# sharph/s-rack

Hardware: AMD Instinct MI355X
Metric: voice-samples/sec @48 kHz offline render (higher is better)
Workload: dtype f32

## Files before the change

### s-rack_amd/csrc/capi.cpp

```cpp
#include <hip/hip_runtime.h>

#include <algorithm>
#include <cmath>
#include <cstdio>
#include <cstring>
#include <mutex>
#include <string>
#include <thread>
#include <vector>

#include "freeverb_params.hpp"
#include "jit.hpp"
#include "runtime.hpp"

using namespace srack;

namespace srack {
int load_srk(const uint8_t* bytes, size_t n_bytes, Graph& g);
std::vector<uint8_t> save_srk(const Graph& g);
}

struct srack_patch {
    PatchHandle h;
};
// ... 1394 lines not shown
int srack_render_info(srack_patch* p, char* buf, size_t cap)
{
    return guarded([&]() -> int {
        CHECK_HANDLE(p);
        int rc = ensure_program(p->h, p->h.prog_valid ? p->h.prog_flags : 0u);
        if (rc != SRACK_OK) return rc;
        std::string s = p->h.prog.description;
        s += tuning_knobs_note();
        const char* k = device_kernel_name(p->h);
        s += device_bus_note(p->h);
        s += device_sends_note(p->h);
        s += device_busvcf_note(p->h);
        s += device_busvca_note(p->h);
        s += device_busfx_note(p->h);
        s += device_master_note(p->h);
        s += device_waves_note(p->h);
        s += device_sequences_note(p->h);
        s += device_jit_note(p->h);
        if (k && *k) s += std::string(" kernel=") + k;
        if (buf && cap) {
            std::strncpy(buf, s.c_str(), cap - 1);
            buf[cap - 1] = 0;
        }
        return (int)s.size();
    });
}

int srack_render_kernel_source(srack_patch* p, uint32_t flags, char* buf, size_t cap)
{
    return guarded([&]() -> int {
// ... 347 lines not shown
```

### s-rack_amd/csrc/chain.hip

```cpp
#include "fused.hip.h"
#include "launch.hpp"

namespace srack {

__global__ __launch_bounds__(64) void render_ctl_gate_env(CtlWork w)
{
    if (w.port & OSC_EXACT)
        ctl_gate_env<true>(w);
    else
        ctl_gate_env<false>(w);
}

void launch_ctl_gate_env(const CtlWork& w, hipStream_t st)
{
    hipLaunchKernelGGL(render_ctl_gate_env, dim3(1), dim3(64), 0, st, w);
}

void launch_fused(uint32_t osc_port, uint32_t vcf_port, bool exact, int out_mode, bool track, const KernelArgs& ka, const ChainRoles& roles, const CtlWork& co,
                  dim3 grid, hipStream_t st)
{
    with_osc_port(osc_port, [&](auto A) { launch_chain<decltype(A)::value>(vcf_port, exact, out_mode, track, ka, roles, co, grid, st); });
}

}
```

### s-rack_amd/csrc/chain_saw.hip

```cpp
#include "chain_unit.hip.h"

namespace srack {
template void launch_chain<OSC_OUT_SAW>(uint32_t, bool, int, bool, const KernelArgs&, const ChainRoles&, const CtlWork&, dim3, hipStream_t);
}
```

### s-rack_amd/csrc/chain_sine.hip

```cpp
#include "chain_unit.hip.h"

namespace srack {
template void launch_chain<OSC_OUT_SINE>(uint32_t, bool, int, bool, const KernelArgs&, const ChainRoles&, const CtlWork&, dim3, hipStream_t);
}
```

### s-rack_amd/csrc/chain_square.hip

```cpp
#include "chain_unit.hip.h"

namespace srack {
template void launch_chain<OSC_OUT_SQUARE>(uint32_t, bool, int, bool, const KernelArgs&, const ChainRoles&, const CtlWork&, dim3, hipStream_t);
}
```

### s-rack_amd/csrc/chain_unit.hip.h

```cpp
#pragma once
#include "fused.hip.h"
#include "launch.hpp"

namespace srack {

template <uint32_t A, uint32_t F, bool E, int O>
static void launch_fused4(bool track, const KernelArgs& ka, const ChainRoles& roles, const CtlWork& co, dim3 grid, hipStream_t st)
{
    if (track)
        hipLaunchKernelGGL((render_voice_chain_track<A, F, E, O>), grid, dim3(64), 0, st, ka, roles, co);
    else
        hipLaunchKernelGGL((render_voice_chain<A, OSC_OUT_SQUARE, F, E, O>), grid, dim3(64), 0, st, ka, roles);
}

template <uint32_t A, uint32_t F>
static void launch_fused3(bool exact, int out_mode, bool track, const KernelArgs& ka, const ChainRoles& roles, const CtlWork& co, dim3 grid, hipStream_t st)
{
    if ((out_mode & kOutStats) && exact)
        launch_fused4<A, F, true, kOutStats>(track, ka, roles, co, grid, st);
    else if (out_mode & kOutStats)
        launch_fused4<A, F, false, kOutStats>(track, ka, roles, co, grid, st);
    else if (exact && out_mode == 3 && track)
        hipLaunchKernelGGL((render_voice_chain_track<A, F, true, 3>), grid, dim3(64), 0, st, ka, roles, co);
    else if (exact)
        launch_fused4<A, F, true, 0>(track, ka, roles, co, grid, st);
    else
        with_out_mode(out_mode, [&](auto O) { launch_fused4<A, F, false, O>(track, ka, roles, co, grid, st); });
}

template <uint32_t kOscAPort>
void launch_chain(uint32_t vcf_port, bool exact, int out_mode, bool track, const KernelArgs& ka, const ChainRoles& roles, const CtlWork& co, dim3 grid, hipStream_t st)
{
#ifdef SRK_WAVE_CENSUS
    if (track) (void)hipMemcpyToSymbolAsync(HIP_SYMBOL(srk_census_rec), census_rec, sizeof(*census_rec), 0, hipMemcpyHostToDevice, st);
#endif
    with_port<VCF_OUT_LP, VCF_OUT_BP, VCF_OUT_HP>(vcf_port, [&](auto F) { launch_fused3<kOscAPort, F>(exact, out_mode, track, ka, roles, co, grid, st); });
}

}
```

### s-rack_amd/csrc/folds.hip.h

```cpp
#pragma once
#include <hip/hip_runtime.h>
#include <type_traits>

#include "kernel_args.hip.h"
#include "modules.hip.h"
#include "wave.hip.h"

namespace srack {

constexpr uint32_t kMixSplit = 16;

struct MixArgs {
    const float* mixpart;
    float* mixgroup;
    float* mix;
    uint32_t T, n_waves, n_channels, n_planes;
    uint32_t mix_stride;
    uint32_t t_begin, t_end;
    int32_t channel_plane[8];
};

__global__ __launch_bounds__(256) void mix_reduce_groups(MixArgs m)
{
    const uint32_t i = m.t_begin + blockIdx.x * 256u + threadIdx.x;
    if (i >= m.t_end) return;
// ... 138 lines not shown
```

### s-rack_amd/csrc/fused.hip.h

```cpp
#pragma once
#include <hip/hip_runtime.h>
#include <type_traits>

#include "kernel_args.hip.h"
#include "launch_types.hpp"
#include "modules.hip.h"
#include "wave.hip.h"

#ifndef SRK_PRIO_AT1
#define SRK_PRIO_AT1 32
#endif
#ifndef SRK_PRIO_AT0
#define SRK_PRIO_AT0 56
#endif


namespace srack {


template <uint32_t kOscPort, bool kExact>
SRK_DEV void ctl_gate_env_body(const CtlWork& a)
{
    using namespace dev;
    const ChainRoles r{0, 0, 0, 1, 0, 2, 0};
    const int lane = threadIdx.x;
    auto row = [&](int rr) { return a.table[rr]; };
    const DevOp& ol = a.ops[r.osc_l];
    const DevOp& od = a.ops[r.adsr];
// ... 234 lines not shown
}
SRK_DEV void census_end(uint32_t* rec)
{
    if (!rec) return;
    const uint64_t t = __builtin_amdgcn_s_memrealtime();
    rec[2] = (uint32_t)t;
    rec[3] = (uint32_t)(t >> 32);
}
SRK_DEV void census_end(uint32_t* rec, const dev::Pace& p)
{
    if (rec && p.word) rec[6] = 1u | 4u | (p.key << 3) | ((p.max_lead < 255u ? p.max_lead : 255u) << 16) | ((p.mine < 255u ? p.mine : 255u) << 24);
    census_end(rec);
}
#endif

template <uint32_t kOscAPort, uint32_t kVcfPort, bool kExact, int kOut>
__global__ __launch_bounds__(64) void render_voice_chain_track(KernelArgs a, ChainRoles r, CtlWork co)
{
    using namespace dev;
    __shared__ __attribute__((aligned(16))) float mix_tile[kMixTile];
    if (blockIdx.x < a.block0) {
        __builtin_amdgcn_s_setprio(3);
#ifdef SRK_WAVE_CENSUS
        uint32_t* crec = census_begin(a.n_waves, 0xffffffffu, true, threadIdx.x);
#endif
        ctl_gate_env<kExact>(co);
#ifdef SRK_WAVE_CENSUS
        census_end(crec);
#endif
        return;
    }
    const int lane = threadIdx.x;
#ifdef SRK_WAVE_CENSUS
    uint32_t* crec = census_begin(blockIdx.x - a.block0, blockIdx.x - a.block0, false, lane);
#endif
    const WaveMap wm = wave_map(a, lane);
    const uint32_t voice = wm.voice, vc = wm.vc, V = a.V;
    const bool active = wm.active;
    auto row = [&](int rr) { return a.table[(size_t)rr * V + vc]; };
    auto parv = [&](const DevOp& op, int k) { return op.par_row[k] >= 0 ? __uint_as_float(row(op.par_row[k])) : op.par_val[k]; };
// ... 194 lines not shown
```

### s-rack_amd/csrc/launch.hpp

```cpp
#pragma once
#include <hip/hip_runtime.h>

#include <cstddef>
#include <cstdint>
#include <type_traits>

#include "kernel_args.hip.h"
#include "launch_types.hpp"

namespace srack {

struct FlatProgram;

enum class Kernel { Interp, VoiceChain, VoiceChainTrack, SeqChain, FmPair, FmPairRing, FmPairSplit, FmPairBlock, FmPairBlockX, FmPairX };

template <class Fn>
static auto with_out_mode(int out_mode, Fn&& f)
{
    switch (out_mode) {
    case 3: return f(std::integral_constant<int, 3>{});
    case 1: return f(std::integral_constant<int, 1>{});
    case 2: return f(std::integral_constant<int, 2>{});
    default: return f(std::integral_constant<int, 0>{});
    }
// ... 4 lines not shown
{
    if (port == P0)
        f(std::integral_constant<uint32_t, P0>{});
    else if (port == P1)
        f(std::integral_constant<uint32_t, P1>{});
    else
        f(std::integral_constant<uint32_t, P2>{});
}
template <class Fn>
static void with_osc_port(uint32_t port, Fn&& f)
{
    with_port<OSC_OUT_SAW, OSC_OUT_SQUARE, OSC_OUT_SINE>(port, f);
}

template <uint32_t kOscAPort>
void launch_chain(uint32_t vcf_port, bool exact, int out_mode, bool track, const KernelArgs& ka, const ChainRoles& roles, const CtlWork& co, dim3 grid, hipStream_t st);
void launch_fused(uint32_t osc_port, uint32_t vcf_port, bool exact, int out_mode, bool track, const KernelArgs& ka, const ChainRoles& roles, const CtlWork& co,
                  dim3 grid, hipStream_t st);
void launch_ctl_gate_env(const CtlWork& w, hipStream_t st);
#ifdef SRK_WAVE_CENSUS
extern uint32_t* const* census_rec;
#endif

void launch_seq(uint32_t osc_port, int out_mode, const KernelArgs& ka, const SeqRoles& r, dim3 grid, hipStream_t st);

void launch_fm_pair(Kernel kernel, bool exact, int out_mode, const KernelArgs& ka, const ChainRoles& roles, dim3 grid, hipStream_t st);
void launch_fm_pair_x(int out_mode, const KernelArgs& ka, const ChainRoles& roles, dim3 grid, hipStream_t st);
hipError_t launch_fm_block(bool x, int out_mode, const KernelArgs& ka, const ChainRoles& roles, hipStream_t st);

inline size_t interp_lds_bytes(const DevProgram& H)
{
    return ((size_t)H.n_rows + 2 + (size_t)H.n_tracks + (size_t)H.n_slots * H.tile) * 256;
}
// ... 13 lines not shown
```

### s-rack_amd/csrc/launch_types.hpp

```cpp
#pragma once
#include <cstdint>

#include "kernel_args.hip.h"

namespace srack {

struct CtlWork {
    const DevOp* ops;
    uint32_t* table;
    float* track;
    uint32_t T;
    uint32_t port;
    uint32_t* table_out;
    uint32_t n_rows;
};

constexpr int kBlkVoices = 32, kBlkSlices = 16, kBlkPer = 16, kBlkChunk = kBlkSlices * kBlkPer;

struct MasterArgs {
    const float* rows;
    const float* gain;
    float* runs;
    float* master;
    double* stats;
    uint32_t n;
    uint32_t n_buses;
    uint32_t row_channels;
    uint32_t used;
};
// ... 77 lines not shown
```

### s-rack_amd/csrc/render.hip

```cpp
#include <hip/hip_runtime.h>

#include <algorithm>
#include <cstdio>
#include <cstdlib>
#include <cstring>
#include <memory>
#include <string>
#include <type_traits>
#include <vector>

#include "busfx.hip.h"
#include "folds.hip.h"
#include "freeverb_params.hpp"
#include "jit.hpp"
#include "kernel_args.hip.h"
#include "launch.hpp"
#include "runtime.hpp"
#include "wave.hip.h"

namespace srack {


#define HIP_TRY(expr)                                                                                   \
    do {                                                                                                \
// ... 3 lines not shown
            return SRACK_ERR_DEVICE;                                                                    \
        }                                                                                               \
    } while (0)

struct Knobs {
    uint32_t want_waves = 1024;
    uint32_t chunk_max = 4096;
    uint32_t chunk_first = 1024;
    bool debug_occ = false;
    int high_prio_ctl = 1;
    int special_ctl = 1;
    int fm_split = 1;
    int fm_block = 1;
    uint32_t fm_block_chunk = 65536;
    uint32_t fm_block_min = 4096;
    int mix_aside = 0;
    int pace = 1;
    int tile_plain = 1;
    int tick = 2;
};
static const Knobs& knobs()
{
    static const Knobs k = [] {
        Knobs v;
        auto num = [](const char* name, long lo, long hi, long dflt) {
            const char* e = getenv(name);
            if (!e || !*e) return dflt;
            char* end = nullptr;
            const long x = strtol(e, &end, 10);
            if (end == e) return dflt;
            return std::min(std::max(x, lo), hi);
        };
        v.want_waves = (uint32_t)num("SRACK_WANT_WAVES", 1, 1 << 20, 1024);
        v.chunk_max = (uint32_t)num("SRACK_CHUNK_MAX", 256, 65536, 4096);
        v.chunk_first = (uint32_t)num("SRACK_CHUNK_FIRST", 32, 4096, 1024);
        v.debug_occ = getenv("SRACK_DEBUG_OCC") != nullptr;
        v.high_prio_ctl = (int)num("SRACK_CTL_HIGH_PRIO", 0, 1, 1);
        v.special_ctl = (int)num("SRACK_SPECIAL_CTL", 0, 1, 1);
        v.fm_split = (int)num("SRACK_FM_SPLIT", 0, 1, 1);
        v.fm_block = (int)num("SRACK_FM_BLOCK", 0, 1, 1);
        v.fm_block_chunk = (uint32_t)num("SRACK_FM_BLOCK_CHUNK", 256, 65536, 65536);
        v.fm_block_min = (uint32_t)num("SRACK_FM_BLOCK_MIN", 1, 65536, 4096);
        v.tick = (int)num("SRACK_TICK", 0, 2, 2);
        v.mix_aside = (int)num("SRACK_MIX_ASIDE", 0, 1, 0);
        v.pace = (int)num("SRACK_PACE", 0, 1, 1);
        v.tile_plain = (int)num("SRACK_TILE_PLAIN", 0, 1, 1);
        return v;
    }();
    return k;
}

struct DevProg {
    DevOp* d_ops = nullptr;
    uint32_t* d_table = nullptr;
    float* d_rings = nullptr;
    uint32_t* d_seqtab = nullptr;
    double* d_fv = nullptr;
    void release()
    {
// ... 21 lines not shown
    uint64_t n0 = 0;
    hipStream_t st = nullptr;
    hipEvent_t done = nullptr;
    float* d_ring = nullptr;
    size_t ring_bytes = 0;
    std::vector<uint32_t*> d_copies;
    std::vector<size_t> words;
    uint64_t slots_base = 0;
    uint32_t slots_n = 0;
};
constexpr uint32_t kPaceSlices = 16;
constexpr uint32_t kTickBatch = 256, kTickFirstBatch = 8;

struct DeviceState {
    TickSession tick;
    hipStream_t mix_stream = nullptr;
    std::vector<hipEvent_t> ev_mix;
    hipEvent_t ev_mix_done = nullptr;
    DevProg voice;
    std::vector<DevProg> ctl;
    KernelArgs* d_stage_slots = nullptr;
    size_t stage_slots_cap = 0;
    std::vector<KernelArgs> h_stage_slots;
    float* d_mixpart = nullptr;
    size_t mixpart_bytes = 0;
    float* d_mixgroup = nullptr;
    size_t mixgroup_bytes = 0;
    float* d_tracks = nullptr;
    size_t tracks_bytes = 0;
    uint32_t* d_pace = nullptr;
    float* d_stat_frames = nullptr;
    size_t stat_frames_bytes = 0;
    uint32_t* d_bus_tab = nullptr;
    uint64_t bus_revision = 0;
    float* d_bus_part = nullptr;
    size_t bus_part_bytes = 0;
    bool last_bank_lds = false;
    uint32_t last_buses = 0;
    std::shared_ptr<const JitKernel> jit[5];
    bool jit_failed = false;
    bool bank_lds[5] = {false, false, false, false, false};
    std::string jit_note;
    std::vector<std::pair<hipEvent_t, hipEvent_t>> timings;
    std::vector<hipEvent_t> pool;
    const char* kernel_name = "";
// ... 6 lines not shown

void device_release(DeviceState* d)
{
    if (!d) return;
    d->voice.release();
    for (DevProg& c : d->ctl) c.release();
    (void)hipFree(d->d_stage_slots);
    (void)hipFree(d->d_mixpart);
    (void)hipFree(d->d_mixgroup);
    (void)hipFree(d->d_tracks);
    (void)hipFree(d->d_pace);
    (void)hipFree(d->d_stat_frames);
    (void)hipFree(d->d_bus_tab);
    (void)hipFree(d->d_bus_part);
    if (d->tick.done) (void)hipEventDestroy(d->tick.done);
    for (hipEvent_t e : d->ev_mix) (void)hipEventDestroy(e);
    if (d->ev_mix_done) (void)hipEventDestroy(d->ev_mix_done);
    if (d->mix_stream) (void)hipStreamDestroy(d->mix_stream);
    (void)hipFree(d->tick.d_ring);
    for (uint32_t* c : d->tick.d_copies) (void)hipFree(c);
    for (auto& p : d->timings) {
        (void)hipEventDestroy(p.first);
        (void)hipEventDestroy(p.second);
    }
    for (auto e : d->pool) (void)hipEventDestroy(e);
    for (auto e : d->ev_chunk) (void)hipEventDestroy(e);
    if (d->ev_begin) (void)hipEventDestroy(d->ev_begin);
    if (d->ev_ready) (void)hipEventDestroy(d->ev_ready);
    if (d->ctl_stream) (void)hipStreamDestroy(d->ctl_stream);
    delete d;
}

PatchHandle::~PatchHandle()
// ... 356 lines not shown
        d->bank_lds[out_mode] = how.bank_lds;
    }
    d->last_bank_lds = d->bank_lds[out_mode];
    *out = d->jit[out_mode].get();
    *with_ctl = ctl;
    pick.name = "render_specialized";
    pick.stats_in_kernel = pick.paced = false;
    if (P.hdr.n_rings == 0 && n_waves <= 1024 && !(flags & SRACK_RENDER_EXACT_OSC)) pick.chunk = std::min(knobs().chunk_max, 2048u);
    return SRACK_OK;
}

static void launch_ctl(const FlatProgram& Cp, const KernelArgs& kc, hipStream_t st)
{
    if (Cp.fused == FUSED_CTL_GATE_ENV) {
        CtlWork w{kc.ops, kc.table, kc.frames + (size_t)Cp.ops[2].aux * kc.plane_stride, kc.T,
                  Cp.ops[0].flags & (OSC_OUT_SINE | OSC_OUT_SQUARE | OSC_OUT_SAW | OSC_EXACT), nullptr, 0u};
        launch_ctl_gate_env(w, st);
    } else if (Cp.fused == FUSED_FM_PAIR) {
        const bool exact = (Cp.render_flags & SRACK_RENDER_EXACT_OSC) != 0;
        launch_fm_pair(fm_pair_kernel(Cp.fused_variant, exact), exact, 1, kc, fm_pair_roles(Cp), dim3(1), st);
    } else {
        launch_interp(Cp, kc, st, knobs().debug_occ);
    }
}

#ifdef SRK_WAVE_CENSUS
static struct {
    uint32_t* d_rec = nullptr;
    uint32_t cap = 0, used = 0;
    std::vector<uint32_t> slots;
    std::vector<uint32_t*> where;
// ... 61 lines not shown
    float* d_bus;
    uint32_t bus_slab = 0;
    const hipStream_t st;
    int rc = SRACK_OK;
    KernelPick pick;
    const uint32_t lanes, n_waves;
    bool has_ctl = false, co_ctl = false, special_ctl = false, tick = false;
    uint32_t n_stages = 0, n_tracks = 0, kChunkMax = 0, kChunkFirst = 0, max_lag = 0, n_chunks = 0, n_ctl_launch = 0;
    uint32_t stride = 0;
    const JitKernel* special = nullptr;
    std::vector<std::pair<uint32_t, uint32_t>> chunks;
    ChainRoles roles{};
    SeqRoles seq{};
    uint32_t osc_port = 0, vcf_port = 0, seq_port = 0;
    MixArgs m{};
    bool mix_aside = false;

    Segment(PatchHandle& h_, uint32_t T_total_, uint32_t t_seg_, uint32_t T_, float* d_frames_, float* d_mix_, double* d_stats_, float* d_bus_, uint32_t flags_, hipStream_t st_)
        : h(h_), P(h_.prog.voice), d(h_.dev), tk(h_.dev->tick), V(h_.prog.voice.n_voices), C((uint32_t)h_.prog.voice.hdr.n_channels), T_total(T_total_),
          t_seg(t_seg_), T(T_), flags(flags_), d_frames(d_frames_ ? d_frames_ + (size_t)t_seg_ * h_.prog.voice.n_voices : nullptr),
          d_mix(d_mix_ ? d_mix_ + t_seg_ : nullptr), d_stats(d_stats_), d_bus(d_bus_ ? d_bus_ + t_seg_ : nullptr), st(st_), pick(pick_kernel(h_.prog, flags_, T_)), lanes(pick.lanes), n_waves((h_.prog.voice.n_voices + lanes - 1) / lanes)
    {
    }

    CtlWork ctl_work(uint32_t t_off, uint32_t len)
    {
        const FlatProgram& Cp = h.prog.ctl[0];
        return CtlWork{d->ctl[0].d_ops, d->ctl[0].d_table, d->d_tracks + (size_t)Cp.ops[2].aux * T + t_off, len,
                       Cp.ops[0].flags & (OSC_OUT_SINE | OSC_OUT_SQUARE | OSC_OUT_SAW | OSC_EXACT), nullptr, 0u};
    }
    int get_event(hipEvent_t& e)
    {
        if (!d->pool.empty()) {
            e = d->pool.back();
            d->pool.pop_back();
            return SRACK_OK;
        }
        HIP_TRY(hipEventCreate(&e));
        return SRACK_OK;
    }

    KernelArgs unit_args(uint32_t s)
    {
        KernelArgs kc{};
// ... 64 lines not shown
        KernelArgs kc = unit_args(s2);
        kc.table = tick_table(s2, x);
        kc.table_out = tick_table(s2, x + 1);
        kc.frames = tick_tracks(x);
        kc.tracks = kc.frames;
        kc.plane_stride = tk.S;
        kc.t_stride = tk.S;
        kc.T = tick_len(x);
        kc.n0 = tick_n0(x);
        return kc;
    }
    CtlWork tick_work(uint64_t x)
    {
        const FlatProgram& Cp = h.prog.ctl[0];
        return CtlWork{d->ctl[0].d_ops, tick_table(0, x), tick_tracks(x) + (size_t)Cp.ops[2].aux * tk.S, tick_len(x),
                       Cp.ops[0].flags & (OSC_OUT_SINE | OSC_OUT_SQUARE | OSC_OUT_SAW | OSC_EXACT), tick_table(0, x + 1), (uint32_t)Cp.hdr.n_rows};
    }
    int tick_upload_slots(uint64_t base)
    {
        const uint32_t fill = max_lag + 1, batch = std::max(base == 0 ? kTickFirstBatch : kTickBatch, tk.n);
        d->h_stage_slots.assign((size_t)(fill + batch) * n_stages, KernelArgs{});
        for (uint32_t s2 = 0; s2 < n_stages; s2++) {
            const uint32_t lag = (uint32_t)h.prog.ctl_lag[s2];
            if (base == 0)
                for (uint32_t g = lag; g < fill; g++) d->h_stage_slots[(size_t)g * n_stages + s2] = tick_unit_args(s2, g - lag);
            for (uint32_t i = 0; i < batch; i++) d->h_stage_slots[(size_t)(fill + i) * n_stages + s2] = tick_unit_args(s2, base + i + fill - lag);
        }
        if ((rc = upload_slots(st)) != SRACK_OK) return rc;
        tk.slots_base = base;
        tk.slots_n = batch;
        return SRACK_OK;
// ... 265 lines not shown
    }

    int voices()
    {
        if (d_mix) {
            m.mixpart = d->d_mixpart;
            m.mixgroup = d->d_mixgroup;
            m.mix = d_mix;
            m.T = stride;
            m.mix_stride = T_total;
            m.n_waves = n_waves;
            m.n_channels = C;
            m.n_planes = (uint32_t)P.hdr.n_planes;
            for (int c = 0; c < 8; c++) m.channel_plane[c] = P.hdr.channel_plane[c];
        }
        mix_aside = d_mix && n_chunks > 1 && knobs().mix_aside;
        if (mix_aside) {
            if (!d->mix_stream) HIP_TRY(hipStreamCreateWithFlags(&d->mix_stream, hipStreamNonBlocking));
            if (!d->ev_mix_done) HIP_TRY(hipEventCreateWithFlags(&d->ev_mix_done, hipEventDisableTiming));
            while (d->ev_mix.size() < n_chunks) {
                hipEvent_t e = nullptr;
                HIP_TRY(hipEventCreateWithFlags(&e, hipEventDisableTiming));
                d->ev_mix.push_back(e);
            }
        }
        const bool paced = pick.paced, exact = (flags & SRACK_RENDER_EXACT_OSC) != 0;
        if (paced && !d->d_pace) HIP_TRY(hipMalloc(&d->d_pace, sizeof(uint32_t) * dev::kPaceKeys * kPaceSlices));
        for (uint32_t k = 0; k < n_chunks; k++) {
            const uint32_t t_off = chunks[k].first, len = chunks[k].second;
            KernelArgs ka{};
            if (paced) {
                if (k % kPaceSlices == 0)
                    HIP_TRY(hipMemsetAsync(d->d_pace, 0, sizeof(uint32_t) * dev::kPaceKeys * std::min(kPaceSlices, n_chunks - k), st));
                ka.pace = d->d_pace + (size_t)(k % kPaceSlices) * dev::kPaceKeys;
            }
            ka.ops = d->voice.d_ops;
            ka.prog = P.hdr;
            ka.table = d->voice.d_table;
            ka.rings = d->voice.d_rings;
            ka.seqtab = d->voice.d_seqtab;
            ka.fv = d->voice.d_fv;
            ka.frames = d_frames ? d_frames + (size_t)t_off * V : nullptr;
            ka.mixpart = d_mix ? d->d_mixpart + t_off : nullptr;
            ka.tracks = tick ? tick_tracks(tk.c + k) : has_ctl ? d->d_tracks + t_off : nullptr;
            ka.plane_stride = (uint64_t)T_total * V;
            ka.t_stride = stride;
            ka.V = V;
            ka.T = len;
            ka.n_waves = n_waves;
// ... 4 lines not shown
            if (fold_rows) {
                ka.frames = d->d_stat_frames;
                ka.plane_stride = (uint64_t)fold_rows * V;
            }
            CtlWork co{};
            if (tick && co_ctl) {
                co = tick_work(tk.c + k + 1);
                ka.block0 = 1;
            } else if (tick) {
                ka.block0 = n_stages;
                ka.ctl_slots = d->d_stage_slots + (size_t)(max_lag + 1 + (tk.c + k - tk.slots_base)) * n_stages;
            } else if (co_ctl && k + 1 < n_chunks) {
                co = ctl_work(chunks[k + 1].first, chunks[k + 1].second);
                ka.block0 = 1;
            }
            if (has_ctl && !co_ctl && !(special && special_ctl)) HIP_TRY(hipStreamWaitEvent(st, d->ev_chunk[k], 0));
            if (!tick && special && special_ctl && k + max_lag + 1 < n_ctl_launch) {
                ka.block0 = n_stages;
                ka.ctl_slots = d->d_stage_slots + (size_t)(k + max_lag + 1) * n_stages;
            }
            hipEvent_t e0 = nullptr, e1 = nullptr;
            const bool timed = h.timing_armed;
            if (timed) {
                if ((rc = get_event(e0)) != SRACK_OK || (rc = get_event(e1)) != SRACK_OK) return rc;
                HIP_TRY(hipEventRecord(e0, st));
            }
            const int out_mode = (ka.frames ? 1 : 0) | (ka.mixpart ? 2 : 0);
            if (special) {
                if ((rc = jit_launch(*special, ka, n_waves + ka.block0, st)) != SRACK_OK) return rc;
            } else {
                switch (pick.kernel) {
                case Kernel::VoiceChainTrack:
#ifdef SRK_WAVE_CENSUS
                    if ((rc = census_arm(n_waves + 1)) != SRACK_OK) return rc;
#endif
                    [[fallthrough]];
                case Kernel::VoiceChain:
                    launch_fused(osc_port, vcf_port, exact, out_mode | (ka.stats ? kOutStats : 0), pick.kernel == Kernel::VoiceChainTrack, ka, roles, co, dim3(n_waves + ka.block0), st);
                    break;
                case Kernel::SeqChain: launch_seq(seq_port, out_mode, ka, seq, dim3(n_waves), st); break;
                case Kernel::FmPairX: launch_fm_pair_x(out_mode, ka, roles, dim3(n_waves), st); break;
                case Kernel::FmPairBlock:
                case Kernel::FmPairBlockX:
                    HIP_TRY(launch_fm_block(pick.kernel == Kernel::FmPairBlockX, out_mode, ka, roles, st));
                    break;
                case Kernel::FmPair:
                case Kernel::FmPairRing:
                case Kernel::FmPairSplit: launch_fm_pair(pick.kernel, exact, out_mode, ka, roles, dim3(n_waves), st); break;
                case Kernel::Interp: launch_interp(P, ka, st, knobs().debug_occ); break;
                }
            }
            HIP_TRY(hipGetLastError());
            if (fold) {
                hipLaunchKernelGGL(stats_fold, dim3((V + 255) / 256, (uint32_t)P.hdr.n_planes), dim3(256), 0, st, ka.frames, ka.plane_stride, V, len, d_stats);
                HIP_TRY(hipGetLastError());
            }
            if (d_bus) {
                const uint32_t n_seg = (uint32_t)h.bus_plan.seg_end.size();
                for (uint32_t r0 = 0; r0 < len; r0 += bus_slab) {
                    const uint32_t rows = std::min(bus_slab, len - r0);
                    const BusFoldArgs b = bus_args(ka.frames + (size_t)r0 * V, ka.plane_stride, t_off + r0, rows);
                    if (n_seg > 0) hipLaunchKernelGGL(bus_fold_tiles, dim3(h.bus_plan.n_tiles, (rows + kBusRows - 1) / kBusRows, (uint32_t)P.hdr.n_planes), dim3(64), 0, st, b);
                    hipLaunchKernelGGL(bus_fold_sum, dim3(h.n_buses * ((rows + 255) / 256)), dim3(256), 0, st, b);
                    HIP_TRY(hipGetLastError());
                }
            }
            if (mix_aside && k + 1 < n_chunks) {
                HIP_TRY(hipEventRecord(d->ev_mix[k], st));
                HIP_TRY(hipStreamWaitEvent(d->mix_stream, d->ev_mix[k], 0));
                MixArgs mk = m;
                mk.t_begin = t_off;
                mk.t_end = t_off + len;
                hipLaunchKernelGGL(mix_reduce_groups, dim3((len + 255) / 256, kMixSplit), dim3(256), 0, d->mix_stream, mk);
                HIP_TRY(hipGetLastError());
            }
            if (timed) {
                HIP_TRY(hipEventRecord(e1, st));
                d->timings.emplace_back(e0, e1);
                if (d->timings.size() > 4096) {
                    d->pool.push_back(d->timings.front().first);
                    d->pool.push_back(d->timings.front().second);
                    d->timings.erase(d->timings.begin());
                }
            }
        }

        return SRACK_OK;
    }

    int mix()
    {
        if (d_mix) {
            m.t_begin = mix_aside ? chunks[n_chunks - 1].first : 0u;
            m.t_end = T;
            hipLaunchKernelGGL(mix_reduce_groups, dim3((m.t_end - m.t_begin + 255) / 256, kMixSplit), dim3(256), 0, st, m);
            if (mix_aside) {
                HIP_TRY(hipEventRecord(d->ev_mix_done, d->mix_stream));
                HIP_TRY(hipStreamWaitEvent(st, d->ev_mix_done, 0));
            }
            hipLaunchKernelGGL(mix_reduce_final, dim3((T + 255) / 256), dim3(256), 0, st, m);
            HIP_TRY(hipGetLastError());
        }
        return SRACK_OK;
    }

    int finish()
    {
        h.samples_rendered += T;
        if (tick) {
            if (!tk.done) HIP_TRY(hipEventCreateWithFlags(&tk.done, hipEventDisableTiming));
            HIP_TRY(hipEventRecord(tk.done, st));
            tk.c += n_chunks;
        }
        return SRACK_OK;
// ... 36 lines not shown
    }
    return Segment(h, T_total, t_seg, T, d_frames, d_mix, d_stats, d_bus, flags, st).run();
}

int device_render(PatchHandle& h, uint32_t n_samples, float* d_frames, float* d_mix, double* d_stats, float* d_bus, uint32_t flags, void* stream)
{
    int rc = ensure_program(h, flags);
    if (rc != SRACK_OK) return rc;
    if (n_samples == 0) return SRACK_OK;
    if (!h.dev) {
        rc = upload_program(h);
        if (rc != SRACK_OK) return rc;
    }
    flags = h.prog.effective_flags | (flags & kLaunchPolicyFlags);
    constexpr uint32_t kSegment = 65536;
    for (uint32_t t = 0; t < n_samples && rc == SRACK_OK; t += kSegment)
        rc = render_segment(h, n_samples, t, std::min(kSegment, n_samples - t), d_frames, d_mix, d_stats, d_bus, flags, (hipStream_t)stream);
    if (h.dev) h.dev->last_buses = d_bus ? h.n_buses : 0u;
    return rc;
}

int device_reserve(PatchHandle& h, uint32_t n_samples, bool want_mix, uint32_t flags)
{
    int rc = ensure_program(h, flags);
    if (rc != SRACK_OK) return rc;
    if (!h.dev) {
        rc = upload_program(h);
        if (rc != SRACK_OK) return rc;
    }
    DeviceState* d = h.dev;
// ... 691 lines not shown
    HIP_TRY(hipGetLastError());
    HIP_TRY(hipEventRecord((hipEvent_t)F.ev_done, st));
    F.last_on = n_on;
    F.last_gated = n_gated;
    F.ran = true;
    return SRACK_OK;
}

std::string device_busvca_note(const PatchHandle& h)
{
    return h.busvca.ran ? " busvca=" + std::to_string(h.busvca.last_on) + "[" + std::to_string(h.busvca.last_gated) + " gated]" : std::string();
}

const char* device_kernel_name(const PatchHandle& h) { return h.dev ? h.dev->kernel_name : ""; }
std::string device_bus_note(const PatchHandle& h) { return h.dev && h.dev->last_buses ? " buses=" + std::to_string(h.dev->last_buses) + "[fold]" : std::string(); }
std::string device_waves_note(const PatchHandle& h)
{
    if (!h.prog_valid || h.prog.n_bank_waves == 0) return std::string();
    const bool lds = h.dev && h.dev->last_bank_lds && std::strncmp(h.dev->kernel_name, "render_specialized", 18) == 0;
    return " waves=" + std::to_string(h.prog.n_bank_waves) + (lds ? "[lds]" : "[global]");
}
std::string device_sequences_note(const PatchHandle& h)
{
    if (!h.prog_valid || h.prog.n_bank_sequences == 0) return std::string();
    return " sequences=" + std::to_string(h.prog.n_bank_sequences) + "[global]";
}
std::string device_jit_note(const PatchHandle& h) { return h.dev ? h.dev->jit_note : std::string(); }

}
```

### s-rack_amd/csrc/runtime.hpp

```cpp
#pragma once
#include <cstdint>
#include <set>
#include <string>
#include <utility>
#include <vector>

#include "buses.hpp"
#include "flatten.hpp"
#include "graph.hpp"

namespace srack {

struct DeviceState;

struct BusFx {
    bool set = false;
    std::vector<double> params;
    std::vector<uint8_t> enabled;
    uint32_t len[kFvLines] = {}, first[kFvLines] = {}, total = 0;
    uint32_t block = 0;
    uint64_t counter = 0;
    std::vector<double*> d_state;
    std::vector<uint8_t> fresh;
    void* d_tab = nullptr;
// ... 138 lines not shown
int device_buses_filter(PatchHandle& h, uint32_t n_samples, const float* d_rows, uint32_t row_channels, const float* d_cv, float* d_out, void* stream);
int device_busvcf_enable(PatchHandle& h, const std::vector<uint8_t>& enabled);
int device_busvcf_state(PatchHandle& h, float* state, uint32_t cap);
void device_busvcf_changed(PatchHandle& h);
void device_busvcf_reset(PatchHandle& h);
void device_busvcf_drop(PatchHandle& h);
std::string device_busvcf_note(const PatchHandle& h);
int device_buses_vca(PatchHandle& h, uint32_t n_samples, const float* d_rows, uint32_t row_channels, const float* d_ctl, float* d_out, float* d_env, void* stream);
int device_busvca_modes(PatchHandle& h, const std::vector<int32_t>& mode);
int device_busvca_state(PatchHandle& h, float* state, uint32_t cap);
void device_busvca_changed(PatchHandle& h);
void device_busvca_reset(PatchHandle& h);
void device_busvca_drop(PatchHandle& h);
std::string device_busvca_note(const PatchHandle& h);
std::string device_bus_note(const PatchHandle& h);
std::string device_waves_note(const PatchHandle& h);
std::string device_sequences_note(const PatchHandle& h);
std::string device_jit_note(const PatchHandle& h);

}
```

Baseline: 1271 billion.

## Fold previous chunk's mix reduction into render kernel tail and clear pace slots in-kernel

Replaces the side-stream mix_reduce_groups launches with extra trailing blocks in the track render kernel. These blocks run at low priority and reduce the previous chunk's mix partials. This mix-tail path sits behind a knob that defaults to off. Separately, the per-chunk hipMemsetAsync of pace slots is replaced with a rotating slot that the control block clears inside the kernel, skipping the memset when the slot is known clean. That pace change is active by default, but it carries a correctness risk if the clean tracking across streams or calls is wrong.

Result: no change. 1271 billion, median of 2 (+0.0%).

```diff
diff --git a/s-rack_amd/csrc/capi.cpp b/s-rack_amd/csrc/capi.cpp
--- a/s-rack_amd/csrc/capi.cpp
+++ b/s-rack_amd/csrc/capi.cpp
@@ -1432,6 +1432,7 @@
         s += device_busvca_note(p->h);
         s += device_busfx_note(p->h);
         s += device_master_note(p->h);
+        s += device_mix_tail_note(p->h);
         s += device_waves_note(p->h);
         s += device_sequences_note(p->h);
         s += device_jit_note(p->h);
diff --git a/s-rack_amd/csrc/chain.hip b/s-rack_amd/csrc/chain.hip
--- a/s-rack_amd/csrc/chain.hip
+++ b/s-rack_amd/csrc/chain.hip
@@ -17,9 +17,9 @@
 }
 
 void launch_fused(uint32_t osc_port, uint32_t vcf_port, bool exact, int out_mode, bool track, const KernelArgs& ka, const ChainRoles& roles, const CtlWork& co,
-                  dim3 grid, hipStream_t st)
+                  const MixTail& tail, dim3 grid, hipStream_t st)
 {
-    with_osc_port(osc_port, [&](auto A) { launch_chain<decltype(A)::value>(vcf_port, exact, out_mode, track, ka, roles, co, grid, st); });
+    with_osc_port(osc_port, [&](auto A) { launch_chain<decltype(A)::value>(vcf_port, exact, out_mode, track, ka, roles, co, tail, grid, st); });
 }
 
 }
diff --git a/s-rack_amd/csrc/chain_saw.hip b/s-rack_amd/csrc/chain_saw.hip
--- a/s-rack_amd/csrc/chain_saw.hip
+++ b/s-rack_amd/csrc/chain_saw.hip
@@ -1,5 +1,5 @@
 #include "chain_unit.hip.h"
 
 namespace srack {
-template void launch_chain<OSC_OUT_SAW>(uint32_t, bool, int, bool, const KernelArgs&, const ChainRoles&, const CtlWork&, dim3, hipStream_t);
+template void launch_chain<OSC_OUT_SAW>(uint32_t, bool, int, bool, const KernelArgs&, const ChainRoles&, const CtlWork&, const MixTail&, dim3, hipStream_t);
 }
diff --git a/s-rack_amd/csrc/chain_sine.hip b/s-rack_amd/csrc/chain_sine.hip
--- a/s-rack_amd/csrc/chain_sine.hip
+++ b/s-rack_amd/csrc/chain_sine.hip
@@ -1,5 +1,5 @@
 #include "chain_unit.hip.h"
 
 namespace srack {
-template void launch_chain<OSC_OUT_SINE>(uint32_t, bool, int, bool, const KernelArgs&, const ChainRoles&, const CtlWork&, dim3, hipStream_t);
+template void launch_chain<OSC_OUT_SINE>(uint32_t, bool, int, bool, const KernelArgs&, const ChainRoles&, const CtlWork&, const MixTail&, dim3, hipStream_t);
 }
diff --git a/s-rack_amd/csrc/chain_square.hip b/s-rack_amd/csrc/chain_square.hip
--- a/s-rack_amd/csrc/chain_square.hip
+++ b/s-rack_amd/csrc/chain_square.hip
@@ -1,5 +1,5 @@
 #include "chain_unit.hip.h"
 
 namespace srack {
-template void launch_chain<OSC_OUT_SQUARE>(uint32_t, bool, int, bool, const KernelArgs&, const ChainRoles&, const CtlWork&, dim3, hipStream_t);
+template void launch_chain<OSC_OUT_SQUARE>(uint32_t, bool, int, bool, const KernelArgs&, const ChainRoles&, const CtlWork&, const MixTail&, dim3, hipStream_t);
 }
diff --git a/s-rack_amd/csrc/chain_unit.hip.h b/s-rack_amd/csrc/chain_unit.hip.h
--- a/s-rack_amd/csrc/chain_unit.hip.h
+++ b/s-rack_amd/csrc/chain_unit.hip.h
@@ -5,36 +5,36 @@
 namespace srack {
 
 template <uint32_t A, uint32_t F, bool E, int O>
-static void launch_fused4(bool track, const KernelArgs& ka, const ChainRoles& roles, const CtlWork& co, dim3 grid, hipStream_t st)
+static void launch_fused4(bool track, const KernelArgs& ka, const ChainRoles& roles, const CtlWork& co, const MixTail& tail, dim3 grid, hipStream_t st)
 {
     if (track)
-        hipLaunchKernelGGL((render_voice_chain_track<A, F, E, O>), grid, dim3(64), 0, st, ka, roles, co);
+        hipLaunchKernelGGL((render_voice_chain_track<A, F, E, O>), grid, dim3(64), 0, st, ka, roles, co, tail);
     else
         hipLaunchKernelGGL((render_voice_chain<A, OSC_OUT_SQUARE, F, E, O>), grid, dim3(64), 0, st, ka, roles);
 }
 
 template <uint32_t A, uint32_t F>
-static void launch_fused3(bool exact, int out_mode, bool track, const KernelArgs& ka, const ChainRoles& roles, const CtlWork& co, dim3 grid, hipStream_t st)
+static void launch_fused3(bool exact, int out_mode, bool track, const KernelArgs& ka, const ChainRoles& roles, const CtlWork& co, const MixTail& tail, dim3 grid, hipStream_t st)
 {
     if ((out_mode & kOutStats) && exact)
-        launch_fused4<A, F, true, kOutStats>(track, ka, roles, co, grid, st);
+        launch_fused4<A, F, true, kOutStats>(track, ka, roles, co, tail, grid, st);
     else if (out_mode & kOutStats)
-        launch_fused4<A, F, false, kOutStats>(track, ka, roles, co, grid, st);
+        launch_fused4<A, F, false, kOutStats>(track, ka, roles, co, tail, grid, st);
     else if (exact && out_mode == 3 && track)
-        hipLaunchKernelGGL((render_voice_chain_track<A, F, true, 3>), grid, dim3(64), 0, st, ka, roles, co);
+        hipLaunchKernelGGL((render_voice_chain_track<A, F, true, 3>), grid, dim3(64), 0, st, ka, roles, co, tail);
     else if (exact)
-        launch_fused4<A, F, true, 0>(track, ka, roles, co, grid, st);
+        launch_fused4<A, F, true, 0>(track, ka, roles, co, tail, grid, st);
     else
-        with_out_mode(out_mode, [&](auto O) { launch_fused4<A, F, false, O>(track, ka, roles, co, grid, st); });
+        with_out_mode(out_mode, [&](auto O) { launch_fused4<A, F, false, O>(track, ka, roles, co, tail, grid, st); });
 }
 
 template <uint32_t kOscAPort>
-void launch_chain(uint32_t vcf_port, bool exact, int out_mode, bool track, const KernelArgs& ka, const ChainRoles& roles, const CtlWork& co, dim3 grid, hipStream_t st)
+void launch_chain(uint32_t vcf_port, bool exact, int out_mode, bool track, const KernelArgs& ka, const ChainRoles& roles, const CtlWork& co, const MixTail& tail, dim3 grid, hipStream_t st)
 {
 #ifdef SRK_WAVE_CENSUS
     if (track) (void)hipMemcpyToSymbolAsync(HIP_SYMBOL(srk_census_rec), census_rec, sizeof(*census_rec), 0, hipMemcpyHostToDevice, st);
 #endif
-    with_port<VCF_OUT_LP, VCF_OUT_BP, VCF_OUT_HP>(vcf_port, [&](auto F) { launch_fused3<kOscAPort, F>(exact, out_mode, track, ka, roles, co, grid, st); });
+    with_port<VCF_OUT_LP, VCF_OUT_BP, VCF_OUT_HP>(vcf_port, [&](auto F) { launch_fused3<kOscAPort, F>(exact, out_mode, track, ka, roles, co, tail, grid, st); });
 }
 
 }
diff --git a/s-rack_amd/csrc/folds.hip.h b/s-rack_amd/csrc/folds.hip.h
--- a/s-rack_amd/csrc/folds.hip.h
+++ b/s-rack_amd/csrc/folds.hip.h
@@ -3,12 +3,12 @@
 #include <type_traits>
 
 #include "kernel_args.hip.h"
+#include "launch_types.hpp"
 #include "modules.hip.h"
 #include "wave.hip.h"
 
 namespace srack {
 
-constexpr uint32_t kMixSplit = 16;
 
 struct MixArgs {
     const float* mixpart;
diff --git a/s-rack_amd/csrc/fused.hip.h b/s-rack_amd/csrc/fused.hip.h
--- a/s-rack_amd/csrc/fused.hip.h
+++ b/s-rack_amd/csrc/fused.hip.h
@@ -12,6 +12,12 @@
 #endif
 #ifndef SRK_PRIO_AT0
 #define SRK_PRIO_AT0 56
+#endif
+#ifndef SRK_TAIL_BATCH
+#define SRK_TAIL_BATCH 24
+#endif
+#ifndef SRK_TRACK_LDS_PAD
+#define SRK_TRACK_LDS_PAD 0
 #endif
 
 
@@ -276,16 +282,55 @@
 }
 #endif
 
+SRK_DEV void mix_tail_block(const MixTail& m, uint32_t b, int lane)
+{
+    const uint32_t y = b / m.n_x, i0 = m.t_begin + (b - y * m.n_x) * 64u;
+    if (y >= kMixSplit || i0 >= m.t_end) return;
+    const uint32_t n = min(64u, m.t_end - i0), lc = min((uint32_t)lane, n - 1u);
+    const uint32_t per = (m.n_waves + kMixSplit - 1) / kMixSplit;
+    const uint32_t w0 = y * per, w1 = min(m.n_waves, w0 + per);
+    for (uint32_t plane = 0; plane < m.n_planes; plane++) {
+        const float* p = m.mixpart + (size_t)plane * m.n_waves * m.T + i0;
+        float s[8] = {0.f, 0.f, 0.f, 0.f, 0.f, 0.f, 0.f, 0.f};
+        uint32_t w = w0;
+        for (; w + SRK_TAIL_BATCH <= w1; w += SRK_TAIL_BATCH) {
+            float v[SRK_TAIL_BATCH];
+#pragma unroll
+            for (int u = 0; u < SRK_TAIL_BATCH; u++) v[u] = p[(size_t)(w + (uint32_t)u) * m.T + lc];
+#pragma unroll
+            for (int u = 0; u < SRK_TAIL_BATCH; u++) s[u & 7] += v[u];
+        }
+        for (; w + 8 <= w1; w += 8) {
+            float v[8];
+#pragma unroll
+            for (int k = 0; k < 8; k++) v[k] = p[(size_t)(w + (uint32_t)k) * m.T + lc];
+#pragma unroll
+            for (int k = 0; k < 8; k++) s[k] += v[k];
+        }
+        for (; w < w1; w++) s[0] += p[(size_t)w * m.T + lc];
+        if ((uint32_t)lane < n) m.mixgroup[((size_t)plane * kMixSplit + y) * m.T + i0 + (uint32_t)lane] = ((s[0] + s[1]) + (s[2] + s[3])) + ((s[4] + s[5]) + (s[6] + s[7]));
+    }
+}
+
 template <uint32_t kOscAPort, uint32_t kVcfPort, bool kExact, int kOut>
-__global__ __launch_bounds__(64) void render_voice_chain_track(KernelArgs a, ChainRoles r, CtlWork co)
+__global__ __launch_bounds__(64) void render_voice_chain_track(KernelArgs a, ChainRoles r, CtlWork co, MixTail tail)
 {
     using namespace dev;
-    __shared__ __attribute__((aligned(16))) float mix_tile[kMixTile];
+    __shared__ __attribute__((aligned(16))) float mix_tile[kMixTile + SRK_TRACK_LDS_PAD];
+    if constexpr (kOut != 1) {
+        if (blockIdx.x >= a.block0 + a.n_waves) {
+            __builtin_amdgcn_s_setprio(0);
+            mix_tail_block(tail, blockIdx.x - a.block0 - a.n_waves, threadIdx.x);
+            return;
+        }
+    }
     if (blockIdx.x < a.block0) {
         __builtin_amdgcn_s_setprio(3);
 #ifdef SRK_WAVE_CENSUS
         uint32_t* crec = census_begin(a.n_waves, 0xffffffffu, true, threadIdx.x);
 #endif
+        if (co.pace_clear)
+            for (uint32_t i = threadIdx.x; i < kPaceKeys / 4u; i += 64u) ((uint4*)co.pace_clear)[i] = make_uint4(0u, 0u, 0u, 0u);
         ctl_gate_env<kExact>(co);
 #ifdef SRK_WAVE_CENSUS
         census_end(crec);
diff --git a/s-rack_amd/csrc/launch.hpp b/s-rack_amd/csrc/launch.hpp
--- a/s-rack_amd/csrc/launch.hpp
+++ b/s-rack_amd/csrc/launch.hpp
@@ -42,9 +42,9 @@
 }
 
 template <uint32_t kOscAPort>
-void launch_chain(uint32_t vcf_port, bool exact, int out_mode, bool track, const KernelArgs& ka, const ChainRoles& roles, const CtlWork& co, dim3 grid, hipStream_t st);
+void launch_chain(uint32_t vcf_port, bool exact, int out_mode, bool track, const KernelArgs& ka, const ChainRoles& roles, const CtlWork& co, const MixTail& tail, dim3 grid, hipStream_t st);
 void launch_fused(uint32_t osc_port, uint32_t vcf_port, bool exact, int out_mode, bool track, const KernelArgs& ka, const ChainRoles& roles, const CtlWork& co,
-                  dim3 grid, hipStream_t st);
+                  const MixTail& tail, dim3 grid, hipStream_t st);
 void launch_ctl_gate_env(const CtlWork& w, hipStream_t st);
 #ifdef SRK_WAVE_CENSUS
 extern uint32_t* const* census_rec;
diff --git a/s-rack_amd/csrc/launch_types.hpp b/s-rack_amd/csrc/launch_types.hpp
--- a/s-rack_amd/csrc/launch_types.hpp
+++ b/s-rack_amd/csrc/launch_types.hpp
@@ -13,6 +13,17 @@
     uint32_t port;
     uint32_t* table_out;
     uint32_t n_rows;
+    uint32_t* pace_clear;
+};
+
+constexpr uint32_t kMixSplit = 16;
+
+struct MixTail {
+    const float* mixpart;
+    float* mixgroup;
+    uint32_t T, n_waves, n_planes;
+    uint32_t t_begin, t_end;
+    uint32_t n_x;
 };
 
 constexpr int kBlkVoices = 32, kBlkSlices = 16, kBlkPer = 16, kBlkChunk = kBlkSlices * kBlkPer;
diff --git a/s-rack_amd/csrc/render.hip b/s-rack_amd/csrc/render.hip
--- a/s-rack_amd/csrc/render.hip
+++ b/s-rack_amd/csrc/render.hip
@@ -41,7 +41,7 @@
     int fm_block = 1;
     uint32_t fm_block_chunk = 65536;
     uint32_t fm_block_min = 4096;
-    int mix_aside = 0;
+    int mix_tail = 0;
     int pace = 1;
     int tile_plain = 1;
     int tick = 2;
@@ -69,7 +69,7 @@
         v.fm_block_chunk = (uint32_t)num("SRACK_FM_BLOCK_CHUNK", 256, 65536, 65536);
         v.fm_block_min = (uint32_t)num("SRACK_FM_BLOCK_MIN", 1, 65536, 4096);
         v.tick = (int)num("SRACK_TICK", 0, 2, 2);
-        v.mix_aside = (int)num("SRACK_MIX_ASIDE", 0, 1, 0);
+        v.mix_tail = (int)num("SRACK_MIX_TAIL", 0, 1, 0);
         v.pace = (int)num("SRACK_PACE", 0, 1, 1);
         v.tile_plain = (int)num("SRACK_TILE_PLAIN", 0, 1, 1);
         return v;
@@ -121,9 +121,6 @@
 
 struct DeviceState {
     TickSession tick;
-    hipStream_t mix_stream = nullptr;
-    std::vector<hipEvent_t> ev_mix;
-    hipEvent_t ev_mix_done = nullptr;
     DevProg voice;
     std::vector<DevProg> ctl;
     KernelArgs* d_stage_slots = nullptr;
@@ -136,6 +133,10 @@
     float* d_tracks = nullptr;
     size_t tracks_bytes = 0;
     uint32_t* d_pace = nullptr;
+    uint32_t pace_next = 0;
+    bool pace_clean = false;
+    hipStream_t pace_stream = nullptr;
+    uint32_t last_mix_tail = 0;
     float* d_stat_frames = nullptr;
     size_t stat_frames_bytes = 0;
     uint32_t* d_bus_tab = nullptr;
@@ -172,9 +173,6 @@
     (void)hipFree(d->d_bus_tab);
     (void)hipFree(d->d_bus_part);
     if (d->tick.done) (void)hipEventDestroy(d->tick.done);
-    for (hipEvent_t e : d->ev_mix) (void)hipEventDestroy(e);
-    if (d->ev_mix_done) (void)hipEventDestroy(d->ev_mix_done);
-    if (d->mix_stream) (void)hipStreamDestroy(d->mix_stream);
     (void)hipFree(d->tick.d_ring);
     for (uint32_t* c : d->tick.d_copies) (void)hipFree(c);
     for (auto& p : d->timings) {
@@ -561,7 +559,7 @@
 {
     if (Cp.fused == FUSED_CTL_GATE_ENV) {
         CtlWork w{kc.ops, kc.table, kc.frames + (size_t)Cp.ops[2].aux * kc.plane_stride, kc.T,
-                  Cp.ops[0].flags & (OSC_OUT_SINE | OSC_OUT_SQUARE | OSC_OUT_SAW | OSC_EXACT), nullptr, 0u};
+                  Cp.ops[0].flags & (OSC_OUT_SINE | OSC_OUT_SQUARE | OSC_OUT_SAW | OSC_EXACT), nullptr, 0u, nullptr};
         launch_ctl_gate_env(w, st);
     } else if (Cp.fused == FUSED_FM_PAIR) {
         const bool exact = (Cp.render_flags & SRACK_RENDER_EXACT_OSC) != 0;
@@ -653,7 +651,7 @@
     SeqRoles seq{};
     uint32_t osc_port = 0, vcf_port = 0, seq_port = 0;
     MixArgs m{};
-    bool mix_aside = false;
+    bool mix_tail = false;
 
     Segment(PatchHandle& h_, uint32_t T_total_, uint32_t t_seg_, uint32_t T_, float* d_frames_, float* d_mix_, double* d_stats_, float* d_bus_, uint32_t flags_, hipStream_t st_)
         : h(h_), P(h_.prog.voice), d(h_.dev), tk(h_.dev->tick), V(h_.prog.voice.n_voices), C((uint32_t)h_.prog.voice.hdr.n_channels), T_total(T_total_),
@@ -666,7 +664,7 @@
     {
         const FlatProgram& Cp = h.prog.ctl[0];
         return CtlWork{d->ctl[0].d_ops, d->ctl[0].d_table, d->d_tracks + (size_t)Cp.ops[2].aux * T + t_off, len,
-                       Cp.ops[0].flags & (OSC_OUT_SINE | OSC_OUT_SQUARE | OSC_OUT_SAW | OSC_EXACT), nullptr, 0u};
+                       Cp.ops[0].flags & (OSC_OUT_SINE | OSC_OUT_SQUARE | OSC_OUT_SAW | OSC_EXACT), nullptr, 0u, nullptr};
     }
     int get_event(hipEvent_t& e)
     {
@@ -761,7 +759,7 @@
     {
         const FlatProgram& Cp = h.prog.ctl[0];
         return CtlWork{d->ctl[0].d_ops, tick_table(0, x), tick_tracks(x) + (size_t)Cp.ops[2].aux * tk.S, tick_len(x),
-                       Cp.ops[0].flags & (OSC_OUT_SINE | OSC_OUT_SQUARE | OSC_OUT_SAW | OSC_EXACT), tick_table(0, x + 1), (uint32_t)Cp.hdr.n_rows};
+                       Cp.ops[0].flags & (OSC_OUT_SINE | OSC_OUT_SQUARE | OSC_OUT_SAW | OSC_EXACT), tick_table(0, x + 1), (uint32_t)Cp.hdr.n_rows, nullptr};
     }
     int tick_upload_slots(uint64_t base)
     {
@@ -1057,25 +1055,23 @@
             m.n_planes = (uint32_t)P.hdr.n_planes;
             for (int c = 0; c < 8; c++) m.channel_plane[c] = P.hdr.channel_plane[c];
         }
-        mix_aside = d_mix && n_chunks > 1 && knobs().mix_aside;
-        if (mix_aside) {
-            if (!d->mix_stream) HIP_TRY(hipStreamCreateWithFlags(&d->mix_stream, hipStreamNonBlocking));
-            if (!d->ev_mix_done) HIP_TRY(hipEventCreateWithFlags(&d->ev_mix_done, hipEventDisableTiming));
-            while (d->ev_mix.size() < n_chunks) {
-                hipEvent_t e = nullptr;
-                HIP_TRY(hipEventCreateWithFlags(&e, hipEventDisableTiming));
-                d->ev_mix.push_back(e);
-            }
-        }
+        mix_tail = d_mix && n_chunks > 1 && knobs().mix_tail && pick.kernel == Kernel::VoiceChainTrack && !special;
         const bool paced = pick.paced, exact = (flags & SRACK_RENDER_EXACT_OSC) != 0;
-        if (paced && !d->d_pace) HIP_TRY(hipMalloc(&d->d_pace, sizeof(uint32_t) * dev::kPaceKeys * kPaceSlices));
+        if (paced && !d->d_pace) {
+            HIP_TRY(hipMalloc(&d->d_pace, sizeof(uint32_t) * dev::kPaceKeys * kPaceSlices));
+            d->pace_clean = false;
+        }
         for (uint32_t k = 0; k < n_chunks; k++) {
             const uint32_t t_off = chunks[k].first, len = chunks[k].second;
             KernelArgs ka{};
+            uint32_t* pace_after = nullptr;
             if (paced) {
-                if (k % kPaceSlices == 0)
-                    HIP_TRY(hipMemsetAsync(d->d_pace, 0, sizeof(uint32_t) * dev::kPaceKeys * std::min(kPaceSlices, n_chunks - k), st));
-                ka.pace = d->d_pace + (size_t)(k % kPaceSlices) * dev::kPaceKeys;
+                ka.pace = d->d_pace + (size_t)d->pace_next * dev::kPaceKeys;
+                if (!d->pace_clean || d->pace_stream != st) HIP_TRY(hipMemsetAsync(ka.pace, 0, sizeof(uint32_t) * dev::kPaceKeys, st));
+                d->pace_next = (d->pace_next + 1) % kPaceSlices;
+                d->pace_clean = false;
+                d->pace_stream = st;
+                pace_after = d->d_pace + (size_t)d->pace_next * dev::kPaceKeys;
             }
             ka.ops = d->voice.d_ops;
             ka.prog = P.hdr;
@@ -1110,6 +1106,13 @@
                 co = ctl_work(chunks[k + 1].first, chunks[k + 1].second);
                 ka.block0 = 1;
             }
+            if (ka.block0 == 1 && co_ctl && !special) co.pace_clear = pace_after;
+            MixTail tail{};
+            if (mix_tail && k > 0) {
+                tail = MixTail{m.mixpart, m.mixgroup, m.T, m.n_waves, m.n_planes, chunks[k - 1].first, chunks[k - 1].first + chunks[k - 1].second,
+                               (chunks[k - 1].second + 63u) / 64u};
+                d->last_mix_tail++;
+            }
             if (has_ctl && !co_ctl && !(special && special_ctl)) HIP_TRY(hipStreamWaitEvent(st, d->ev_chunk[k], 0));
             if (!tick && special && special_ctl && k + max_lag + 1 < n_ctl_launch) {
                 ka.block0 = n_stages;
@@ -1132,7 +1135,8 @@
 #endif
                     [[fallthrough]];
                 case Kernel::VoiceChain:
-                    launch_fused(osc_port, vcf_port, exact, out_mode | (ka.stats ? kOutStats : 0), pick.kernel == Kernel::VoiceChainTrack, ka, roles, co, dim3(n_waves + ka.block0), st);
+                    launch_fused(osc_port, vcf_port, exact, out_mode | (ka.stats ? kOutStats : 0), pick.kernel == Kernel::VoiceChainTrack, ka, roles, co, tail,
+                                 dim3(n_waves + ka.block0 + tail.n_x * kMixSplit), st);
                     break;
                 case Kernel::SeqChain: launch_seq(seq_port, out_mode, ka, seq, dim3(n_waves), st); break;
                 case Kernel::FmPairX: launch_fm_pair_x(out_mode, ka, roles, dim3(n_waves), st); break;
@@ -1147,6 +1151,7 @@
                 }
             }
             HIP_TRY(hipGetLastError());
+            if (co.pace_clear) d->pace_clean = true;
             if (fold) {
                 hipLaunchKernelGGL(stats_fold, dim3((V + 255) / 256, (uint32_t)P.hdr.n_planes), dim3(256), 0, st, ka.frames, ka.plane_stride, V, len, d_stats);
                 HIP_TRY(hipGetLastError());
@@ -1161,15 +1166,6 @@
                     HIP_TRY(hipGetLastError());
                 }
             }
-            if (mix_aside && k + 1 < n_chunks) {
-                HIP_TRY(hipEventRecord(d->ev_mix[k], st));
-                HIP_TRY(hipStreamWaitEvent(d->mix_stream, d->ev_mix[k], 0));
-                MixArgs mk = m;
-                mk.t_begin = t_off;
-                mk.t_end = t_off + len;
-                hipLaunchKernelGGL(mix_reduce_groups, dim3((len + 255) / 256, kMixSplit), dim3(256), 0, d->mix_stream, mk);
-                HIP_TRY(hipGetLastError());
-            }
             if (timed) {
                 HIP_TRY(hipEventRecord(e1, st));
                 d->timings.emplace_back(e0, e1);
@@ -1187,13 +1183,9 @@
     int mix()
     {
         if (d_mix) {
-            m.t_begin = mix_aside ? chunks[n_chunks - 1].first : 0u;
+            m.t_begin = mix_tail ? chunks[n_chunks - 1].first : 0u;
             m.t_end = T;
             hipLaunchKernelGGL(mix_reduce_groups, dim3((m.t_end - m.t_begin + 255) / 256, kMixSplit), dim3(256), 0, st, m);
-            if (mix_aside) {
-                HIP_TRY(hipEventRecord(d->ev_mix_done, d->mix_stream));
-                HIP_TRY(hipStreamWaitEvent(st, d->ev_mix_done, 0));
-            }
             hipLaunchKernelGGL(mix_reduce_final, dim3((T + 255) / 256), dim3(256), 0, st, m);
             HIP_TRY(hipGetLastError());
         }
@@ -1260,6 +1252,7 @@
     }
     flags = h.prog.effective_flags | (flags & kLaunchPolicyFlags);
     constexpr uint32_t kSegment = 65536;
+    h.dev->last_mix_tail = 0;
     for (uint32_t t = 0; t < n_samples && rc == SRACK_OK; t += kSegment)
         rc = render_segment(h, n_samples, t, std::min(kSegment, n_samples - t), d_frames, d_mix, d_stats, d_bus, flags, (hipStream_t)stream);
     if (h.dev) h.dev->last_buses = d_bus ? h.n_buses : 0u;
@@ -1981,6 +1974,7 @@
 
 const char* device_kernel_name(const PatchHandle& h) { return h.dev ? h.dev->kernel_name : ""; }
 std::string device_bus_note(const PatchHandle& h) { return h.dev && h.dev->last_buses ? " buses=" + std::to_string(h.dev->last_buses) + "[fold]" : std::string(); }
+std::string device_mix_tail_note(const PatchHandle& h) { return h.dev && h.dev->last_mix_tail ? " mix_tail=" + std::to_string(h.dev->last_mix_tail) : std::string(); }
 std::string device_waves_note(const PatchHandle& h)
 {
     if (!h.prog_valid || h.prog.n_bank_waves == 0) return std::string();
diff --git a/s-rack_amd/csrc/runtime.hpp b/s-rack_amd/csrc/runtime.hpp
--- a/s-rack_amd/csrc/runtime.hpp
+++ b/s-rack_amd/csrc/runtime.hpp
@@ -176,6 +176,7 @@
 void device_busvca_drop(PatchHandle& h);
 std::string device_busvca_note(const PatchHandle& h);
 std::string device_bus_note(const PatchHandle& h);
+std::string device_mix_tail_note(const PatchHandle& h);
 std::string device_waves_note(const PatchHandle& h);
 std::string device_sequences_note(const PatchHandle& h);
 std::string device_jit_note(const PatchHandle& h);
```
